# eldenpark/halo2-pse

Hardware: AMD Instinct MI355X
Metric: bn254_msm_g1_adds_per_sec (higher is better)
Workload: dtype u32x8 (256-bit Montgomery integers)

## Files before the change

### halo2-pse_amd/csrc/api.hip

```cpp
#include <dlfcn.h>
#include <rccl/rccl.h>
#include <stdarg.h>
#include <stdlib.h>
#include <string.h>

#include <atomic>
#include <condition_variable>
#include <deque>
#include <functional>
#include <shared_mutex>
#include <thread>

#include "../../include/halo2hip.h"
#include "../../include/halo2hip_debug.h"
#include "engine.h"

extern "C" {
static void lazy_forget(const void* key);
static void lazy_reset();
static void lazy_pin_consider(const uint64_t* bases_xy, size_t n);
}

namespace h2 {

static thread_local char g_err[512] = "";

void set_error(const char* fmt, ...) {
    va_list ap;
    va_start(ap, fmt);
    vsnprintf(g_err, sizeof(g_err), fmt, ap);
    va_end(ap);
}

int DevBuf::ensure(size_t bytes) {
    if (bytes <= cap) return 0;
    if (p) {
        H2_CHECK(hipDeviceSynchronize());
        H2_CHECK(hipFree(p));
// ... 169 lines not shown
            for (auto& w : mask_ac) w = 0xffffffffu;
            for (auto& w : mask_b) w = 0xffffffffu;
        }
        H2_CHECK(hipExtStreamCreateWithCUMask(&aux1, words, mask_ac.data()));
        H2_CHECK(hipExtStreamCreateWithCUMask(&aux2, words, mask_ac.data()));
        H2_CHECK(hipExtStreamCreateWithCUMask(&aux_b, words, mask_b.data()));
        aux_reserved = K;
    }
    while (aux_events.size() < n_events) {
        hipEvent_t e;
        H2_CHECK(hipEventCreateWithFlags(&e, hipEventDisableTiming));
        aux_events.push_back(e);
    }
    return 0;
}

struct Config {
    size_t multi_gpu_min_n = (size_t)1 << 18;
    size_t msm_min_n = (size_t)1 << 10;
    uint32_t ntt_min_log_n = 10;
    bool gather_rccl = false;
    bool fixed_base = true;
    size_t table_max_bytes = (size_t)160 << 30;
    bool allow_dup = false;
    bool roctx = false;
    uint32_t lazy_pin_after = 0;
    size_t column_cache_bytes = (size_t)64 << 30;
};
static Config g_cfg;

static bool env_u64(const char* name, uint64_t* out) {
    const char* v = getenv(name);
    if (!v || !*v) return false;
    char* end = nullptr;
    unsigned long long x = strtoull(v, &end, 0);
    if (end == v) return false;
    *out = x;
    return true;
}

static void read_config() {
    Config c;
    uint64_t v;
    if (env_u64("HALO2_HIP_MULTI_GPU_MIN_N", &v)) c.multi_gpu_min_n = (size_t)v;
    if (env_u64("HALO2_HIP_MSM_MIN_N", &v)) c.msm_min_n = (size_t)v;
    if (env_u64("HALO2_HIP_NTT_MIN_LOGN", &v)) c.ntt_min_log_n = (uint32_t)v;
    if (env_u64("HALO2_HIP_FIXED_BASE", &v)) c.fixed_base = v != 0;
    if (env_u64("HALO2_HIP_TABLE_MAX_GB", &v)) c.table_max_bytes = (size_t)v << 30;
    if (env_u64("HALO2_HIP_ALLOW_DUPLICATE_DEVICES", &v)) c.allow_dup = v != 0;
    if (env_u64("HALO2_HIP_ROCTX", &v)) c.roctx = v != 0;
    if (env_u64("HALO2_HIP_LAZY_PIN", &v)) c.lazy_pin_after = (uint32_t)v;
    if (env_u64("HALO2_HIP_COLUMN_CACHE_GB", &v)) c.column_cache_bytes = (size_t)v << 30;
    if (env_u64("HALO2_HIP_NTT_TWIDDLE_MB", &v)) ntt_set_full_twiddle_budget(v << 20);
    if (env_u64("HALO2_HIP_EVALH_CODEGEN", &v)) evalh_debug_set_codegen((int)v, 0);
    if (env_u64("HALO2_HIP_MSM_WINDOW", &v) && v >= 2 && v <= 24) msm_set_window((uint32_t)v);
    {
        uint64_t on = 1, min_n = 0;
        const bool has_on = env_u64("HALO2_HIP_STREAM", &on), has_min = env_u64("HALO2_HIP_STREAM_MIN_N", &min_n);
        if (has_on || has_min) msm_set_stream(has_on && on == 0 ? 1 : 0, 0.0, has_min ? (size_t)min_n : 0);
    }
    const char* g = getenv("HALO2_HIP_GATHER");
    if (g && !strcmp(g, "rccl")) c.gather_rccl = true;
    g_cfg = c;
}

static int (*g_roctx_push)(const char*) = nullptr;
static int (*g_roctx_pop)() = nullptr;
static void roctx_load() {
    if (g_roctx_push) return;
    void* h = dlopen("libroctx64.so.4", RTLD_NOW | RTLD_GLOBAL);
    if (!h) h = dlopen("libroctx64.so", RTLD_NOW | RTLD_GLOBAL);
    if (!h) return;
    g_roctx_push = (int (*)(const char*))dlsym(h, "roctxRangePushA");
    g_roctx_pop = (int (*)())dlsym(h, "roctxRangePop");
    if (!g_roctx_push || !g_roctx_pop) g_roctx_push = nullptr, g_roctx_pop = nullptr;
}

struct Rccl {
// ... 631 lines not shown
            const size_t i = pin_sample_index(total, k);
            if (i < n) ok = memcmp(it->second.sample + 64 * k, bases_xy + 8 * i, 64) == 0;
        }
    }
    if (!ok) {
        ::lazy_forget((const void*)bases_xy);
        (void)unpin_everywhere((const void*)bases_xy);
        return true;
    }
    return n == total || n > pin_sample_index(total, 3);
}

__global__ void pin_sample_kernel(const Affine* __restrict__ src, size_t total, Affine* __restrict__ out) {
    if (threadIdx.x < H2_PIN_SAMPLES) out[threadIdx.x] = src[pin_sample_index(total, threadIdx.x)];
}

static const MsmTable* pinned_table(Ctx* c, const void* key, size_t n, MsmTable* out, const PinnedBases** entry) {
    auto it = c->pinned.find(key);
    if (it == c->pinned.end() || !it->second.device_key || n > it->second.n || !it->second.c) return nullptr;
    out->table = (const Affine*)it->second.d;
    out->stride = it->second.n;
    out->c = it->second.c;
    out->W = it->second.W;
    *entry = &it->second;
    return out;
}

static int msm_device_keyed(Ctx* c, const Fe* const* d_scalars, const Affine* d_bases, size_t n, size_t count, XYZZ* out, hipStream_t s) {
    MsmTable tab;
    const PinnedBases* pb = nullptr;
    const MsmTable* t = (n && count) ? pinned_table(c, d_bases, n, &tab, &pb) : nullptr;
    if (t && n != pb->n && n <= pin_sample_index(pb->n, 3)) t = nullptr;
    volatile uint32_t* flag = nullptr;
    if (t && pb->d_sample) {
        int rc = c->pin_flag.ensure(64);
        if (rc) return rc;
        flag = (volatile uint32_t*)c->pin_flag.p;
        *flag = 0;
        c->pin_chk.bases = d_bases;
        c->pin_chk.samples = (const Affine*)pb->d_sample;
        c->pin_chk.flag = (uint32_t*)c->pin_flag.p;
        c->pin_chk.n = n;
        c->pin_chk.total = pb->n;
    }
    int rc = msm_batch_device(c, d_scalars, false, d_bases, n, count, out, s, t);
    c->pin_chk = Ctx::PinCheck();
// ... 103 lines not shown
    const Fe* sc = (const Fe*)d_scalars;
    int rc = msm_device_keyed(en.c, &sc, (const Affine*)d_bases_xy, n, 1, &r, s);
    if (rc) return rc;
    xyzz_to_out(r, out_xyz);
    return 0;
}

static int msm_shard_host(Ctx* c, const uint64_t* const* scalars, const uint64_t* bases_xy, size_t lo, size_t n, size_t count, XYZZ* out,
                          bool use_cache = true) {
    std::vector<const Fe*> sc(count);
    for (size_t j = 0; j < count; j++) sc[j] = (const Fe*)scalars[j] + lo;
    MsmTable tab;
    const Affine *d_bases = nullptr, *h_bases = nullptr;
    const MsmTable* t = nullptr;
    auto it = c->pinned.find((const void*)bases_xy);
    if (use_cache && it != c->pinned.end() && it->second.lo <= lo && lo + n <= it->second.hi) {
        const PinnedBases& pb = it->second;
        d_bases = (const Affine*)pb.d + (lo - pb.lo);
        if (pb.c) {
            tab.table = d_bases;
            tab.stride = pb.n;
            tab.c = pb.c;
            tab.W = pb.W;
            t = &tab;
        }
    } else {
        h_bases = (const Affine*)bases_xy + lo;
    }
    return msm_batch_device(c, sc.data(), true, d_bases, n, count, out, c->stream, t, h_bases);
}

static void fold_host(int n_use, size_t count, const std::vector<std::vector<XYZZ>>& parts, uint64_t* out_xyz) {
    for (size_t j = 0; j < count; j++) {
        XYZZ acc = xyzz_identity();
        for (int d = 0; d < n_use; d++) xyzz_add(acc, parts[(size_t)d][j]);
        xyzz_to_out(acc, out_xyz + 12 * j);
    }
}

static int gather_rccl(size_t count, std::vector<XYZZ>* all) {
    const int nd = (int)g_devs.size();
    const size_t bytes = count * sizeof(XYZZ);
    if (g_rccl.comms.size() != (size_t)nd || bytes > H2_GATHER_OWN) return H2HIP_EINVAL;
    ncclResult_t nr = g_rccl.GroupStart();
    for (int d = 0; nr == ncclSuccess && d < nd; d++) {
        Ctx* x = g_devs[(size_t)d];
// ... 129 lines not shown
    if (rc) return rc;
    for (size_t j = 0; j < count; j++) xyzz_to_out(r[j], out_xyz + 12 * j);
    return 0;
}

static int pin_on_device(Ctx* c, const void* key, const uint64_t* h_points, const void* d_src, size_t lo, size_t hi, size_t n_total,
                         const uint8_t* sample, bool device_key) {
    (void)n_total;
    auto it = c->pinned.find(key);
    if (it != c->pinned.end()) {
        H2_CHECK(hipDeviceSynchronize());
        (void)hipFree(it->second.d);
        if (it->second.d_sample) (void)hipFree(it->second.d_sample);
        c->pinned.erase(it);
    }
    if (hi <= lo) return 0;
    const size_t n = hi - lo;
    PinnedBases pb;
    pb.n = n;
    pb.lo = lo;
    pb.hi = hi;
    pb.device_key = device_key;
    if (sample) memcpy(pb.sample, sample, sizeof(pb.sample));
    uint32_t cw = 0, W = 1;
    if (g_cfg.fixed_base && n <= ((size_t)1 << 26)) {
        cw = msm_table_window(n);
        W = (255 + cw - 1) / cw;
        if ((size_t)W * n * sizeof(Affine) > g_cfg.table_max_bytes) cw = 0, W = 1;
    }
    hipError_t e = hipMalloc(&pb.d, (size_t)W * n * sizeof(Affine));
    if (e != hipSuccess && cw) {
        (void)hipGetLastError();
        cw = 0;
        W = 1;
        e = hipMalloc(&pb.d, n * sizeof(Affine));
    }
    if (e != hipSuccess) {
        set_error("bases_pin: hipMalloc(%zu) failed: %s", (size_t)W * n * sizeof(Affine), hipGetErrorString(e));
        return H2HIP_ENOMEM;
    }
    int rc = 0;
    if (d_src) {
        if (!cw) H2_CHECK(hipMemcpyAsync(pb.d, (const Affine*)d_src + lo, n * sizeof(Affine), hipMemcpyDeviceToDevice, c->stream));
    } else {
        H2_CHECK(hipMemcpyAsync(pb.d, (const Affine*)h_points + lo, n * sizeof(Affine), hipMemcpyHostToDevice, c->stream));
    }
    if (cw) rc = msm_table_build(c, d_src ? (const Affine*)d_src + lo : (const Affine*)pb.d, n, cw, (Affine*)pb.d, c->stream);
    if (!rc && device_key) {
        if (hipMalloc(&pb.d_sample, H2_PIN_SAMPLES * sizeof(Affine)) != hipSuccess) {
            (void)hipGetLastError();
            pb.d_sample = nullptr;
            set_error("bases_pin: hipMalloc of the fingerprint failed");
            rc = H2HIP_ENOMEM;
        } else {
            hipLaunchKernelGGL(pin_sample_kernel, dim3(1), dim3(64), 0, c->stream, (const Affine*)d_src + lo, n, (Affine*)pb.d_sample);
        }
    }
    if (!rc && hipStreamSynchronize(c->stream) != hipSuccess) {
        set_error("bases_pin: table build failed");
        rc = H2HIP_EDEVICE;
    }
    if (rc) {
        (void)hipFree(pb.d);
        if (pb.d_sample) (void)hipFree(pb.d_sample);
        return rc;
    }
    pb.c = cw;
    pb.W = cw ? W : 0;
    c->pinned[key] = pb;
    return 0;
}

static void pin_sample(const uint64_t* bases_xy, size_t n, uint8_t* out) {
    for (uint32_t k = 0; k < H2_PIN_SAMPLES; k++) memcpy(out + 64 * k, bases_xy + 8 * pin_sample_index(n, k), 64);
}

static int pin_host_everywhere(const uint64_t* bases_xy, size_t n) {
    uint8_t sample[H2_PIN_SAMPLES * 64];
    pin_sample(bases_xy, n, sample);
    const int nd = (int)g_devs.size();
    const int use = n >= g_cfg.multi_gpu_min_n ? nd : 1;
    const size_t per = n / (size_t)use;
    int rc = on_devices(nd, [&](int d) -> int {
        size_t lo = d < use ? (size_t)d * per : n, hi = d < use ? (d == use - 1 ? n : (size_t)(d + 1) * per) : n;
        return pin_on_device(g_devs[(size_t)d], (const void*)bases_xy, bases_xy, nullptr, lo, hi, n, sample, false);
    });
    if (rc) (void)unpin_everywhere((const void*)bases_xy);
    return rc;
}

int h2hip_bases_pin(const uint64_t* bases_xy, size_t n) {
// ... 147 lines not shown
        return 0;
    });
    if (rc) return rc;
    std::vector<XYZZ> all;
    if ((rc = gather_rccl(count, &all))) return rc;
    std::vector<std::vector<XYZZ>> parts((size_t)nd, std::vector<XYZZ>(count));
    for (int d = 0; d < nd; d++)
        for (size_t j = 0; j < count; j++) parts[(size_t)d][j] = all[(size_t)d * count + j];
    fold_host(nd, count, parts, out_xyz);
    return 0;
}

int h2hip_bases_pinned_info(const void* bases_xy, size_t* n_points, uint32_t* window_bits, uint32_t* windows, size_t* device_bytes) {
    Entry en(nullptr, nullptr, true);
    if (en.rc) return en.rc;
    size_t n = 0, bytes = 0;
    uint32_t c = 0, W = 0;
    bool found = false;
    for (Ctx* x : g_devs) {
        auto it = x->pinned.find(bases_xy);
        if (it == x->pinned.end()) continue;
        found = true;
        n += it->second.n;
        bytes += (size_t)(it->second.c ? it->second.W : 1) * it->second.n * sizeof(Affine);
        if (it->second.c) c = it->second.c, W = it->second.W;
    }
    if (!found) {
        set_error("bases_pinned_info: pointer is not pinned");
        return H2HIP_EINVAL;
    }
    if (n_points) *n_points = n;
    if (window_bits) *window_bits = c;
    if (windows) *windows = W;
    if (device_bytes) *device_bytes = bytes;
    return 0;
}

int h2hip_g1_fold(const uint64_t* partials_xyz, size_t k, uint64_t out_xyz[12]) {
    if (!out_xyz || (k && !partials_xyz)) {
        set_error("g1_fold: null argument");
        return H2HIP_EINVAL;
    }
    XYZZ acc = xyzz_identity();
    for (size_t i = 0; i < k; i++) {
        Jac j;
        memcpy(&j, partials_xyz + 12 * i, 96);
        xyzz_add(acc, jac_to_xyzz(j));
    }
// ... 590 lines not shown
        return H2HIP_EINVAL;
    }
    Entry en("h2hip_gen_scalars_device", d_out);
    if (en.rc) return en.rc;
    return gen_scalars_device(seed, start, n, (Fe*)d_out, (hipStream_t)stream);
}

int h2hip_gen_points_device(uint64_t seed, uint64_t start, size_t n, void* d_out, void* stream) {
    if (n && !d_out) {
        set_error("gen_points: null output");
        return H2HIP_EINVAL;
    }
    Entry en("h2hip_gen_points_device", d_out);
    if (en.rc) return en.rc;
    return gen_points_device(seed, start, n, (Affine*)d_out, (hipStream_t)stream);
}

int h2hip_set_msm_window(uint32_t c) {
    if (c != 0 && (c < 2 || c > 24)) {
        set_error("msm window must be 0 (auto) or 2..24");
        return H2HIP_EINVAL;
    }
    msm_set_window(c);
    return 0;
}

uint32_t h2hip_get_msm_window(size_t n) { return msm_get_window(n); }
uint32_t h2hip_get_msm_window_fixed_base(size_t n) { return msm_table_window(n); }

int h2hip_debug_set_msm_max_chunk(size_t m) {
    msm_set_max_chunk(m);
    return 0;
}

int h2hip_debug_set_msm_stream(uint32_t chunks, uint32_t ratio_permille, size_t min_n) {
    msm_set_stream(chunks, ratio_permille / 1000.0, min_n);
    return 0;
}

size_t h2hip_debug_msm_stream_ladder(size_t n, uint32_t chunks, uint32_t ratio_permille, int with_bases, size_t* sizes, size_t cap) {
    if (!sizes && cap) return 0;
    return msm_debug_ladder(n, chunks, ratio_permille / 1000.0, with_bases != 0, sizes, cap);
}

int h2hip_debug_set_msm_heavy_div(size_t d) {
    msm_set_heavy_div(d);
    return 0;
}

int h2hip_debug_set_g2l_quad(int on) {
    ecfft_set_quad(on != 0);
// ... 167 lines not shown
```

### halo2-pse_amd/csrc/engine.h

```cpp
#pragma once
#include <hip/hip_runtime.h>
#include <stdint.h>
#include <stdio.h>
#include <string.h>

#include <map>
#include <mutex>
#include <shared_mutex>
#include <string>
#include <vector>

#include "../../include/halo2hip.h"
#include "ecu.h"

namespace h2 {

void set_error(const char* fmt, ...);

#define H2_CHECK(expr)                                                                             \
    do {                                                                                           \
        hipError_t _e = (expr);                                                                    \
        if (_e != hipSuccess) {                                                                    \
            h2::set_error("%s:%d: %s -> %s", __FILE__, __LINE__, #expr, hipGetErrorString(_e));    \
            return 2;                                                                              \
// ... 21 lines not shown
        for (int i = 0; i < 8; i++)
            if (omega[i] != o.omega[i]) return omega[i] < o.omega[i];
        return log_n < o.log_n;
    }
};

struct TwiddleTable {
    Fu* lo = nullptr;
    Fu* hi = nullptr;
    uint32_t lo_bits = 0;
    Fu* stage_of[13] = {};
#define H2_TW_FULL 12
    Fu* full[H2_TW_FULL] = {};
    uint32_t full_tag[H2_TW_FULL] = {};
    Fe full_scale[H2_TW_FULL] = {};
    Fu* lo_scaled = nullptr;
    Fe lo_scale;
};

struct MsmTable {
    const Affine* table = nullptr;
    size_t stride = 0;
    uint32_t c = 0, W = 0;
};

#define H2_GATHER_OWN ((size_t)64 << 10)
#define H2_PIN_SAMPLES 16
static inline __host__ __device__ size_t pin_sample_index(size_t total, uint32_t k) { return k == 0 ? 0 : (total - 1) >> (H2_PIN_SAMPLES - 1 - k); }
struct PinnedBases {
    void* d = nullptr;
    size_t n = 0;
    uint32_t c = 0, W = 0;
    bool device_key = false;
    uint8_t sample[H2_PIN_SAMPLES * 64];
    void* d_sample = nullptr;
    size_t lo = 0, hi = 0;
};

struct Ctx;

#define H2_COL_SAMPLES 16
struct PinnedColumn {
    void* d = nullptr;
    size_t elems = 0;
    uint64_t last_use = 0;
    uint8_t sample[H2_COL_SAMPLES * 32];
};

struct StageTimer {
    std::string name;
    hipEvent_t e0 = nullptr, e1 = nullptr;
    double total_ms = 0.0;
    uint64_t count = 0;
    bool pending = false;
};
// ... 287 lines not shown
```

### halo2-pse_amd/csrc/msm.hip

```cpp
#include <hip/hip_ext.h>
#include <string.h>

#include <atomic>
#include <condition_variable>
#include <thread>
#include <vector>

#include "ecq.h"
#include "engine.h"
#include "host64.h"

namespace h2 {

#define MSM_MAX_C1 1024u
#define MSM_MAX_L 12u
#define MSM_STAGE 16384u
#define MSM_COUNT_TILE 4096u

struct MsmPlan {
    uint32_t c;
    uint32_t W;
    uint32_t q;
    uint32_t cb;
    uint32_t NB;
    uint32_t shared;
    uint32_t heavy_t;
    uint32_t chunk;
};

template <class F>
__device__ __forceinline__ void for_each_digit(const Fe& s, uint32_t c, uint32_t q, uint32_t W, F&& f) {
    uint64_t buf = 0;
    uint32_t nb = 0, w = 0, carry = 0;
    uint32_t width = q ? c : c - 1;
    auto emit = [&]() {
        uint32_t d = ((uint32_t)buf & ((1u << width) - 1)) + carry;
        uint32_t neg = 0;
        carry = 0;
        if (d > (1u << (width - 1))) {
            d = (1u << width) - d;
            neg = 1;
            carry = 1;
        }
        if (d) f(w, d - 1, neg);
        w++;
        buf >>= width;
        nb = nb > width ? nb - width : 0;
        width = w < q ? c : c - 1;
    };
#pragma unroll
    for (int limb = 0; limb < 8; limb++) {
        buf |= (uint64_t)s.l[limb] << nb;
        nb += 32;
        while (nb >= width && w < W) emit();
    }
    while (w < W) emit();
}

struct L1Args {
    const Fe* scalars_one;
    const Fe* const* list;
    uint32_t n, c, q, W, cb, L, C1;
    uint32_t shared, stride;
    uint32_t tile;
    uint16_t* tile_hist;
    const uint32_t* tile_off;
    uint2* tmp;
    uint32_t* tmp_e;
    uint16_t* tmp_k;
    const Affine* chk_bases;
    const Affine* chk_samples;
    uint32_t* chk_flag;
    size_t chk_n, chk_total;
};

__device__ __forceinline__ Fe fr_to_canonical(const Fe& x) {
    Fu c32 = fu_zero();
    c32.l[0] = 32;
    return fu_mul_canon<FrU>(fu_slice(x), c32);
}

#define MSM_TCHUNK 64u
#ifndef MSM_SCATTER_XG
#define MSM_SCATTER_XG 4u
#endif

__global__ void __launch_bounds__(256) msm_l1_count_kernel(L1Args a) {
    __shared__ uint32_t lh[MSM_MAX_C1];
    if (a.chk_flag && blockIdx.x == 0 && blockIdx.y == 0 && threadIdx.x < 4 * H2_PIN_SAMPLES) {
        const uint32_t k = threadIdx.x >> 2, part = threadIdx.x & 3;
        const size_t idx = pin_sample_index(a.chk_total, k);
        if (idx < a.chk_n) {
            const uint4 u = reinterpret_cast<const uint4*>(&a.chk_bases[idx])[part], v = reinterpret_cast<const uint4*>(&a.chk_samples[k])[part];
            if (u.x != v.x || u.y != v.y || u.z != v.z || u.w != v.w) atomicOr(a.chk_flag, 1u);
        }
    }
    for (uint32_t b = threadIdx.x; b < a.C1; b += 256) lh[b] = 0;
    __syncthreads();
    const Fe* __restrict__ scalars = a.list ? a.list[blockIdx.y] : a.scalars_one;
    const uint32_t set0 = a.shared ? blockIdx.y : blockIdx.y * a.W;
    for (uint32_t t = threadIdx.x; t < a.tile; t += 256) {
        const uint32_t i = blockIdx.x * a.tile + t;
        if (i < a.n) {
            const Fe sc = fr_to_canonical(scalars[i]);
            for_each_digit(sc, a.c, a.q, a.W, [&](uint32_t w, uint32_t slot, uint32_t) {
                const uint32_t gb = ((set0 + (a.shared ? 0u : w)) << a.cb) | slot;
                atomicAdd(&lh[gb >> a.L], 1u);
            });
        }
    }
    __syncthreads();
    uint16_t* row = a.tile_hist + (size_t)(blockIdx.y * gridDim.x + blockIdx.x) * a.C1;
    for (uint32_t b = threadIdx.x; b < a.C1; b += 256) row[b] = (uint16_t)lh[b];
}

__global__ void __launch_bounds__(256) msm_l1_chunk_kernel(const uint16_t* __restrict__ tile_hist, uint32_t n_tiles, uint32_t C1,
                                                           uint32_t* __restrict__ chunk_sum) {
    const uint32_t b = blockIdx.y * 256 + threadIdx.x;
    if (b >= C1) return;
    const uint32_t t0 = blockIdx.x * MSM_TCHUNK, t1 = t0 + MSM_TCHUNK < n_tiles ? t0 + MSM_TCHUNK : n_tiles;
    uint32_t sum = 0;
#pragma unroll 8
    for (uint32_t t = t0; t < t1; t++) sum += tile_hist[(size_t)t * C1 + b];
    chunk_sum[(size_t)blockIdx.x * C1 + b] = sum;
}

template <int BS>
__device__ __forceinline__ uint32_t block_scan_base(const uint32_t* cnt, uint32_t n, uint32_t per, uint32_t* ps, uint32_t* total) {
// ... 33 lines not shown
    uint32_t tx = blockIdx.x;
    if (XG && tx < (gridDim.x & ~((8u << XG) - 1))) {
        const uint32_t q = tx >> (3 + XG), r = tx & ((8u << XG) - 1);
        tx = ((q * 8 + (r & 7)) << XG) | (r >> 3);
    }
    const size_t row = (size_t)(blockIdx.y * gridDim.x + tx) * a.C1;
    for (uint32_t b = threadIdx.x; b < a.C1; b += 1024) cur[b] = a.tile_hist[row + b];
    const Fe* __restrict__ scalars = a.list ? a.list[blockIdx.y] : a.scalars_one;
    const uint32_t set0 = a.shared ? blockIdx.y : blockIdx.y * a.W;
    const uint32_t i = tx * a.tile + threadIdx.x;
    const bool live = threadIdx.x < a.tile && i < a.n;
    Fe sc;
    if (live) sc = fr_to_canonical(scalars[i]);
    __syncthreads();
    uint32_t total;
    uint32_t run = block_scan_base<1024>(cur, a.C1, 1, ps, &total);
    if (threadIdx.x < a.C1) {
        const uint32_t b = threadIdx.x;
        delta[b] = a.tile_off[row + b] - run;
        cur[b] = run;
    }
    __syncthreads();
    if (live) {
        for_each_digit(sc, a.c, a.q, a.W, [&](uint32_t w, uint32_t slot, uint32_t neg) {
            const uint32_t gb = ((set0 + (a.shared ? 0u : w)) << a.cb) | slot;
            const uint32_t pos = atomicAdd(&cur[gb >> a.L], 1u);
            stage[pos] = make_uint2((a.shared ? w * a.stride + i : i) | (neg << 31), gb);
        });
    }
    __syncthreads();
    for (uint32_t pos = threadIdx.x; pos < total; pos += 1024) {
        const uint2 e = stage[pos];
        const uint32_t at = pos + delta[e.y >> a.L];
        if (SPLIT) {
            a.tmp_e[at] = e.x;
            a.tmp_k[at] = (uint16_t)(e.y & ((1u << a.L) - 1));
        } else {
            a.tmp[at] = e;
        }
    }
}

__global__ void __launch_bounds__(1024) msm_l1_scan_kernel(uint32_t* __restrict__ chunk_sum, uint32_t n_chunks, uint32_t C1,
                                                           uint32_t* __restrict__ bin_total, uint32_t* __restrict__ zero, uint32_t zero_words) {
    __shared__ uint32_t part_sum[16][64];
    if (blockIdx.x == 0)
        for (uint32_t i = threadIdx.x; i < zero_words; i += 1024) zero[i] = 0;
    const uint32_t lb = threadIdx.x & 63, p = threadIdx.x >> 6, b = blockIdx.x * 64 + lb;
    const uint32_t per = (n_chunks + 15) / 16, c0 = p * per, c1 = c0 + per < n_chunks ? c0 + per : n_chunks;
    uint32_t sum = 0;
// ... 517 lines not shown
    }
    if (live && g == 0) J.out[task] = sh[threadIdx.x];
}

struct FinalArr {
    const XYZZu* base;
    uint32_t stride;
    uint32_t len;
    uint32_t o, k;
    uint32_t nbits;
};
struct FinalArgs {
    FinalArr arr[4];
    uint32_t n_arr;
};

__global__ void __launch_bounds__(256) msm_final_kernel(FinalArgs args, XYZZ* __restrict__ set_sums) {
    __shared__ XYZZu sh[256];
    const uint32_t set = blockIdx.x, ai = threadIdx.x >> 6, v = threadIdx.x & 63;
    XYZZu x = xyzzu_identity();
    if (ai < args.n_arr) {
        const FinalArr& A = args.arr[ai];
        if (v < A.len) {
            const uint32_t wgt = (v + A.o) << A.k;
            if (wgt) x = xyzzu_mul_small(A.base[(size_t)set * A.stride + v], wgt, A.nbits);
        }
    }
    XYZZu r = block_tree_sum(x, sh);
    if (threadIdx.x == 0) set_sums[set] = xyzzu_to_ext(r);
}


__global__ void __launch_bounds__(64) msm_rowcol_quad_kernel(RowColArgs args) {
    __shared__ XYZZu sh[16];
    uint32_t ji = 0;
    for (uint32_t q = 1; q < args.n_jobs; q++)
        if (blockIdx.x >= args.job[q].first_block) ji = q;
    const RowColJob& J = args.job[ji];
    const uint32_t quad = threadIdx.x >> 2, role = threadIdx.x & 3;
    const uint32_t G = 1u << J.g_log, g = quad & (G - 1);
    const uint32_t rows = 1u << J.log_rows, cols = 1u << J.log_cols;
    const uint32_t per_arr = J.cols_kind ? cols : rows;
    const uint32_t task = (blockIdx.x - J.first_block) * (16u >> J.g_log) + (quad >> J.g_log);
    const bool live = task < J.n_arr * per_arr;
    XYZZu acc = xyzzu_identity();
    if (live) {
        const uint32_t a = task / per_arr, idx = task - a * per_arr;
// ... 26 lines not shown
    const uint32_t set = blockIdx.x / n_groups, group = blockIdx.x - set * n_groups;
    const uint32_t quad = threadIdx.x >> 2, role = threadIdx.x & 3;
    uint32_t e = group * 16 + quad;
    const XYZZu* base = nullptr;
    uint32_t stride = 0, o = 0, k = 0, nbits = 0;
    bool found = false;
#pragma unroll
    for (uint32_t i = 0; i < 4; i++) {
        if (i < args.n_arr && !found) {
            if (e < args.arr[i].len) {
                found = true;
                base = args.arr[i].base;
                stride = args.arr[i].stride;
                o = args.arr[i].o;
                k = args.arr[i].k;
                nbits = args.arr[i].nbits;
            } else {
                e -= args.arr[i].len;
            }
        }
    }
    XYZZu x = xyzzu_identity();
    if (found) {
        const uint32_t wgt = (e + o) << k;
        if (wgt) x = xyzzu_mul_small_q(base[(size_t)set * stride + e], wgt, nbits, role);
    }
    if (role == 0) sh[quad] = x;
    __syncthreads();
    for (uint32_t st = 8; st >= 1; st >>= 1) {
        if (quad < st) {
            XYZZu a = sh[quad];
            xyzzu_add_q(a, sh[quad + st], role);
            if (role == 0) sh[quad] = a;
        }
        __syncthreads();
    }
    if (n_groups == 1) {
        if (threadIdx.x == 0) set_sums[set] = xyzzu_to_ext(sh[0]);
        return;
    }
    if (threadIdx.x == 0) {
        partials[blockIdx.x] = sh[0];
        __threadfence();
        is_last = atomicAdd(&done[set], 1u) == n_groups - 1;
    }
    __syncthreads();
    if (!is_last) return;
// ... 18 lines not shown
struct PlaneJob {
    const XYZZu* base;
    uint32_t log_len;
    uint32_t o;
    uint32_t n_planes;
    uint32_t wgs;
    uint32_t first_plane;
    uint32_t first_block;
};
struct PlaneArgs {
    PlaneJob job[2];
    uint32_t blocks_per_set, planes_per_set;
};

__global__ void __launch_bounds__(256) msm_planes_kernel(PlaneArgs args, XYZZu* __restrict__ partials, uint32_t* __restrict__ done,
                                                         XYZZ* __restrict__ plane_sums) {
    __shared__ XYZZu sh[64];
    __shared__ uint32_t is_last;
    const uint32_t set = blockIdx.x / args.blocks_per_set, b = blockIdx.x - set * args.blocks_per_set;
    const PlaneJob& J = args.job[b >= args.job[1].first_block ? 1 : 0];
    const uint32_t pb = b - J.first_block, plane = pb / J.wgs, part = pb - plane * J.wgs;
    const XYZZu* X = J.base + ((size_t)set << J.log_len);
    const uint32_t quad = threadIdx.x >> 2, role = threadIdx.x & 3;
    const bool top = plane == J.log_len;
    const uint32_t count = top ? 1u : 1u << (J.log_len - 1);
    auto elem = [&](uint32_t t) -> XYZZu {
        if (t >= count) return xyzzu_identity();
        const uint32_t v = top ? (1u << J.log_len) : ((t >> plane) << (plane + 1)) | (1u << plane) | (t & ((1u << plane) - 1));
        return X[v - J.o];
    };
    const uint32_t t0 = part * 128 + 2 * quad;
    const XYZZu x = xyzzu_sum_q(elem(t0), elem(t0 + 1), role);
    if (role == 0) sh[quad] = x;
    __syncthreads();
    for (uint32_t st = 32; st >= 1; st >>= 1) {
        if (quad < st) {
            const XYZZu a = xyzzu_sum_q(sh[quad], sh[quad + st], role);
            if (role == 0) sh[quad] = a;
        }
        __syncthreads();
    }
    const uint32_t out = set * args.planes_per_set + J.first_plane + plane;
    if (J.wgs == 1) {
        if (threadIdx.x == 0) plane_sums[out] = xyzzu_to_ext(sh[0]);
        return;
    }
    if (threadIdx.x == 0) {
        partials[(size_t)out * 16 + part] = sh[0];
        __threadfence();
        is_last = atomicAdd(&done[out], 1u) == J.wgs - 1;
    }
    __syncthreads();
    if (!is_last) return;
    __builtin_amdgcn_fence(__ATOMIC_ACQUIRE, "agent");
    XYZZu y = xyzzu_identity();
// ... 63 lines not shown
    if (lg <= 8) return 7;
    if (lg <= 12) return 10;
    if (lg <= 14) return 13;
    if (lg <= 17) return 15;
    return 17;
}

static uint32_t normalise_window(uint32_t c) {
    if (c < 2) c = 2;
    if (c > 22) c = 22;
    const uint32_t W = (255 + c - 1) / c;
    return (255 + W - 1) / W;
}

uint32_t msm_table_window(size_t n) {
    if (g_window_override) return normalise_window(g_window_override);
    const uint32_t lg = floor_log2(n);
    uint32_t c = lg <= 12 ? 13 : lg <= 17 ? 17 : lg <= 21 ? 20 : 22;
    return normalise_window(c);
}

static MsmPlan make_plan(size_t n, bool fused, const MsmTable* tab, uint32_t force_c = 0) {
    MsmPlan p;
    uint32_t c = tab ? tab->c : force_c ? force_c : plain_window(n, fused);
    if (c < 2) c = 2;
    if (c > 24) c = 24;
    p.W = (255 + c - 1) / c;
    c = (255 + p.W - 1) / p.W;
    p.c = c;
    p.q = 255 - p.W * (c - 1);
    p.cb = c - 1;
    p.NB = 1u << (c - 1);
    p.shared = tab ? 1 : 0;
    size_t t = (n * p.W) / g_heavy_div;
    if (t < 32) t = 32;
    const size_t mean = (p.shared ? n * p.W : n) >> p.cb;
    if (t < 8 * mean) t = 8 * mean;
    p.heavy_t = (uint32_t)t;
    p.chunk = 1024;
    return p;
}

uint32_t msm_get_window(size_t n) { return make_plan(n, false, nullptr).c; }

static XYZZ combine_windows(const XYZZ* ws, const MsmPlan& p) {
    h64::P acc = h64::identity();
// ... 22 lines not shown
    MsmPlan p;
    size_t n, E;
    uint32_t K;
    uint32_t L, C1, bin_shift;
    uint32_t tile, tiles_x, n_tiles, n_tchunks;
    uint32_t split_log;
    uint32_t levels, s, rb, s2, s3;
    size_t max_chunks, max_heavy;
    size_t o_zero, o_zero_end, o_bintot, o_hist, o_hcnt, o_fdone, o_cstart, o_tmp, o_vals, o_start, o_counts, o_perm, o_buckets, o_parts, o_RA, o_CA, o_RR,
        o_RC, o_CR, o_CC, o_sums, o_partials, o_ppart, o_hb, o_hc, o_hs, o_ptrs, o_thist, o_toff, o_chsum, total;
};

static int msm_layout(size_t n, MsmLayout* L, uint32_t fuse, const MsmTable* tab, uint32_t force_c = 0, int force_split = -1) {
    MsmPlan p = make_plan(n, fuse > 1, tab, force_c);
    L->p = p;
    L->n = n;
    L->fuse = fuse;
    L->n_sets = p.shared ? fuse : fuse * p.W;
    L->E = n * p.W * fuse;
    if (L->E >= ((size_t)1 << 31)) {
        set_error("msm: %zu entries exceed the 2^31 limit of one run (window override too small?)", L->E);
        return 1;
    }
    if (p.shared && (uint64_t)p.W * tab->stride >= (1ull << 31)) {
        set_error("msm: fixed-base table index exceeds 31 bits");
        return 1;
    }
    const uint64_t K64 = (uint64_t)L->n_sets << p.cb;
    if (K64 > ((uint64_t)MSM_MAX_C1 << MSM_MAX_L)) {
        set_error("msm: too many buckets (%llu) for one run", (unsigned long long)K64);
        return 1;
    }
    L->K = (uint32_t)K64;
    uint32_t want = 1;
    while (want < MSM_MAX_C1 && (size_t)want * g_bin_entries < L->E) want <<= 1;
    uint32_t Lb = 0;
    while (Lb < p.cb && Lb < MSM_MAX_L && (K64 >> Lb) > want) Lb++;
    while ((K64 >> Lb) > MSM_MAX_C1) {
        if (Lb >= p.cb || Lb >= MSM_MAX_L) {
            set_error("msm: too many bucket sets (%u) for one run", L->n_sets);
            return 1;
        }
        Lb++;
    }
    L->L = Lb;
    L->C1 = (uint32_t)(K64 >> Lb);
    L->tile = (MSM_STAGE / p.W) & ~63u;
// ... 58 lines not shown
    const MsmPlan& p = L.p;
    const size_t n = L.n;
    uint32_t* cstart = (uint32_t*)(base + L.o_cstart);
    uint32_t *vals = (uint32_t*)(base + L.o_vals), *start = (uint32_t*)(base + L.o_start);
    uint32_t *counts = (uint32_t*)(base + L.o_counts), *perm = (uint32_t*)(base + L.o_perm);
    int t0 = c->timer_begin("msm_digits", s);
    L1Args a;
    a.scalars_one = d_scalars_list[0];
    a.list = nullptr;
    if (L.fuse > 1) {
        int rc = c->stage_h2d(base + L.o_ptrs, d_scalars_list, L.fuse * sizeof(void*), s);
        if (rc) return rc;
        a.list = (const Fe* const*)(base + L.o_ptrs);
    }
    a.n = (uint32_t)n;
    a.c = p.c;
    a.q = p.q;
    a.W = p.W;
    a.cb = p.cb;
    a.L = L.L;
    a.C1 = L.C1;
    a.shared = p.shared;
    a.stride = tab ? (uint32_t)tab->stride : 0;
    a.tile = L.tile;
    a.tile_hist = (uint16_t*)(base + L.o_thist);
    a.tile_off = (const uint32_t*)(base + L.o_toff);
    a.tmp = (uint2*)(base + L.o_tmp);
    a.chk_bases = c->pin_chk.bases;
    a.chk_samples = c->pin_chk.samples;
    a.chk_flag = c->pin_chk.flag;
    a.chk_n = c->pin_chk.n;
    a.chk_total = c->pin_chk.total;
    c->pin_chk = Ctx::PinCheck();
    uint32_t* chsum = (uint32_t*)(base + L.o_chsum);
    const dim3 tiles(L.tiles_x, L.fuse), chunks(L.n_tchunks, (L.C1 + 255) / 256);
    hipLaunchKernelGGL(msm_l1_count_kernel, tiles, dim3(256), 0, s, a);
    H2_CHECK(hipGetLastError());
    c->timer_end(t0, s);
    int t1 = c->timer_begin("msm_sort", s);
    hipLaunchKernelGGL(msm_l1_chunk_kernel, chunks, dim3(256), 0, s, (const uint16_t*)a.tile_hist, L.n_tiles, L.C1, chsum);
    H2_CHECK(hipGetLastError());
    uint32_t* bin_total = (uint32_t*)(base + L.o_bintot);
    hipLaunchKernelGGL(msm_l1_scan_kernel, dim3((L.C1 + 63) / 64), dim3(1024), 0, s, chsum, L.n_tchunks, L.C1, bin_total,
                       (uint32_t*)(base + L.o_zero), (uint32_t)((L.o_zero_end - L.o_zero) / 4));
    H2_CHECK(hipGetLastError());
    hipLaunchKernelGGL(msm_l1_offsets_kernel, chunks, dim3(256), 0, s, (const uint16_t*)a.tile_hist, L.n_tiles, L.C1, (const uint32_t*)chsum,
// ... 77 lines not shown
        j->log_cols = log_cols;
        j->cols_kind = kind;
        j->g_log = g_log;
        j->first_block = *n_blocks;
        const uint64_t tasks = (uint64_t)n_arr << log_sums;
        const uint32_t per_block = (quad ? 16u : 256u) >> g_log;
        *n_blocks += (uint32_t)((tasks + per_block - 1) / per_block);
    }
}

static bool g_plane_tail = true;
void msm_set_plane_tail(bool on) { g_plane_tail = on; }
static bool msm_plane_tail(const Ctx* c, const MsmLayout& L) {
    return g_plane_tail && g_quad_tail && L.levels >= 1 && L.n_sets <= MSM_PLANE_SETS_MAX && L.rb <= 11 && L.s <= 11 && L.rb >= 1 && L.s >= 1 &&
           L.s + 1 + L.rb <= MSM_PLANES_MAX && !c->gather_want;
}
static inline uint32_t msm_planes_per_set(const MsmLayout& L) { return L.rb + L.s + 1; }

static void msm_planes_finish(const MsmLayout& L, const XYZZ* planes, XYZZ* sums) {
    const uint32_t pps = msm_planes_per_set(L);
    for (uint32_t set = 0; set < L.n_sets; set++) {
        const XYZZ* P = planes + (size_t)set * pps;
        h64::P acc = h64::identity();
        for (uint32_t m = L.s + L.rb; m-- > 0;) {
            acc = h64::pdouble(acc);
            if (m >= L.s) h64::padd(acc, h64::from_xyzz(P[L.s + 1 + (m - L.s)]));
            if (m <= L.s) h64::padd(acc, h64::from_xyzz(P[m]));
        }
        sums[set] = h64::to_xyzz(acc);
    }
}

static int msm_stage_c(Ctx* c, const MsmLayout& L, char* base, XYZZ* h_sums, hipStream_t s, XYZZ* h_planes = nullptr) {
    XYZZu* buckets = (XYZZu*)(base + L.o_buckets);
    XYZZu *RA = (XYZZu*)(base + L.o_RA), *CA = (XYZZu*)(base + L.o_CA), *RR = (XYZZu*)(base + L.o_RR), *RC = (XYZZu*)(base + L.o_RC);
    XYZZu *CR = (XYZZu*)(base + L.o_CR), *CC = (XYZZu*)(base + L.o_CC);
    const bool direct = !c->gather_want;
    XYZZ* sums = direct ? h_sums : (XYZZ*)(base + L.o_sums);
    const uint32_t ns = L.n_sets, cb = L.p.cb;
    const bool quad = g_quad_tail && ns <= 64;
    int t4 = c->timer_begin("msm_reduce", s);
    FinalArgs fa;
    memset(&fa, 0, sizeof(fa));
    auto set_arr = [&](uint32_t i, const XYZZu* b, uint32_t log_len, uint32_t o, uint32_t k) {
        fa.arr[i].base = b;
        fa.arr[i].stride = 1u << log_len;
        fa.arr[i].len = 1u << log_len;
        fa.arr[i].o = o;
        fa.arr[i].k = k;
        fa.arr[i].nbits = bits_of(((1u << log_len) - 1 + o) << k);
    };
    if (L.levels == 0) {
        set_arr(0, buckets, cb, 1, 0);
        fa.n_arr = 1;
    } else {
        RowColArgs ra;
        memset(&ra, 0, sizeof(ra));
        uint32_t nblk = 0;
        rowcol_jobs(&ra, buckets, RA, CA, ns, L.rb, L.s, &nblk);
        if (g_rowcol_qtree)
            hipLaunchKernelGGL(msm_rowcol_qtree_kernel<FqUA>, dim3(nblk), dim3(256), 0, s, ra);
        else if (g_rowcol_asm)
            hipLaunchKernelGGL(msm_rowcol_kernel<FqUA>, dim3(nblk), dim3(256), 0, s, ra);
        else
            hipLaunchKernelGGL(msm_rowcol_kernel<FqU>, dim3(nblk), dim3(256), 0, s, ra);
        H2_CHECK(hipGetLastError());
        if (h_planes && msm_plane_tail(c, L)) {
            PlaneArgs pa;
            memset(&pa, 0, sizeof(pa));
            uint32_t blk = 0, pl = 0;
            for (uint32_t k = 0; k < 2; k++) {
                PlaneJob& J = pa.job[k];
                J.base = k ? RA : CA;
                J.log_len = k ? L.rb : L.s;
                J.o = k ? 0 : 1;
                J.n_planes = J.log_len + J.o;
                J.wgs = J.log_len > 7 ? 1u << (J.log_len - 8) : 1;
                J.first_plane = pl;
                J.first_block = blk;
                pl += J.n_planes;
                blk += J.n_planes * J.wgs;
            }
            pa.blocks_per_set = blk;
            pa.planes_per_set = pl;
            hipLaunchKernelGGL(msm_planes_kernel, dim3(ns * blk), dim3(256), 0, s, pa, (XYZZu*)(base + L.o_ppart), (uint32_t*)(base + L.o_fdone), h_planes);
            H2_CHECK(hipGetLastError());
            c->timer_end(t4, s);
            return 0;
        }
        if (L.levels == 1) {
            set_arr(0, RA, L.rb, 0, L.s);
            set_arr(1, CA, L.s, 1, 0);
            fa.n_arr = 2;
        } else {
            memset(&ra, 0, sizeof(ra));
            nblk = 0;
            rowcol_jobs(&ra, RA, RR, RC, ns, L.rb - L.s2, L.s2, &nblk, quad);
            rowcol_jobs(&ra, CA, CR, CC, ns, L.s - L.s3, L.s3, &nblk, quad);
            if (quad)
// ... 443 lines not shown
```

### include/halo2hip_debug.h

```cpp
#ifndef HALO2HIP_DEBUG_H
#define HALO2HIP_DEBUG_H
#include "halo2hip.h"

#ifdef __cplusplus
extern "C" {
#endif

int h2hip_debug_set_msm_stream(uint32_t chunks, uint32_t ratio_permille, size_t min_n);
size_t h2hip_debug_msm_stream_ladder(size_t n, uint32_t chunks, uint32_t ratio_permille, int with_bases, size_t* sizes, size_t cap);
int h2hip_debug_set_msm_max_chunk(size_t m);
int h2hip_debug_rccl_gather_selftest(const uint64_t* partials_xyz, size_t count, uint64_t* out_xyz);
int h2hip_debug_set_msm_heavy_div(size_t d);
int h2hip_debug_set_g2l_quad(int on);
int h2hip_debug_set_msm_fuse_limits(size_t entries, size_t max_n);
int h2hip_debug_set_msm_rowcol(uint64_t lanes, int use_asm);
int h2hip_debug_set_msm_split_buckets(int on);
int h2hip_debug_set_msm_plane_tail(int on);
int h2hip_debug_set_msm_quad_tail(int on);
int h2hip_debug_set_msm_bucket_order(int local);
int h2hip_debug_set_msm_split_records(int on);
int h2hip_debug_set_msm_bin_entries(size_t d);
int h2hip_debug_set_reserved_cus(uint32_t k);
int h2hip_debug_set_msm_fuse_small(int on);
int h2hip_debug_set_ntt_smax(uint32_t v);
int h2hip_debug_ntt_plan(uint32_t log_n, size_t count, uint32_t radices[4]);
int h2hip_debug_set_lazy_pin(uint32_t after);
int h2hip_debug_set_ntt_two_pass(uint32_t lo, uint32_t hi);
int h2hip_debug_set_ntt_twiddle_budget(uint64_t bytes);
int h2hip_debug_set_ntt_batch_bytes(uint64_t bytes);
int h2hip_debug_set_ntt_two_pass_batch_wgs(uint64_t v);
int h2hip_debug_set_ntt_full_max_log_m(uint32_t v);
int h2hip_debug_set_ntt_fold_tables(int on);
int h2hip_debug_set_ntt_host_batch(uint64_t run_bytes, uint64_t group_bytes);
int h2hip_debug_set_ntt_two_pass_log_j(int v);
int h2hip_debug_set_evalh_max_local_slots(uint32_t v);
int h2hip_debug_set_evalh_lookup_group_bytes(uint64_t v);
int h2hip_debug_evalh_program_muls(const h2hip_graph* g, uint32_t* n_mul);
int h2hip_debug_set_evalh_codegen(int mode, uint32_t max_ops);
int h2hip_debug_evalh_codegen_source(const h2hip_graph* g, char* buf, size_t cap, size_t* len, int compile, double* seconds, size_t* code_bytes);
int h2hip_debug_evalh_codegen_stats(uint64_t out[5]);
int h2hip_debug_evalh_compile_stats(const h2hip_graph* g, uint32_t* n_ops, uint32_t* n_slots);
int h2hip_debug_set_opening_tile(uint32_t rows_per_thread, uint32_t threads_per_tile);
int h2hip_debug_set_lookup_sort(uint32_t lds_keys);
int h2hip_debug_lookup_sort_stats(uint32_t out[2]);
// ... 7 lines not shown
```

Before: 11.59 billion.

## Add per-bit fixed-base table with sliding-window NAF digit decomposition for MSM

For pinned bases with n between 2^19 and 2^23, a 255-row table of 2^k·P is built and scalars are recoded as signed odd-digit sliding-window NAF. Each nonzero digit maps to a bucket by its odd magnitude and to a table row by its bit position. All digits share one bucket set of 2^(w-2) odd buckets with width 20 by default, and the final bucket reduction and plane kernels are adjusted for odd weights. This aims to cut the number of bucket adds per scalar by skipping zero runs and to shrink the reduction, but it costs a much larger table in memory and allocation, with more gather traffic.

```diff
diff --git a/halo2-pse_amd/csrc/api.hip b/halo2-pse_amd/csrc/api.hip
--- a/halo2-pse_amd/csrc/api.hip
+++ b/halo2-pse_amd/csrc/api.hip
@@ -14,6 +14,7 @@
 #include "../../include/halo2hip.h"
 #include "../../include/halo2hip_debug.h"
 #include "engine.h"
+#include "msm_naf.h"
 
 extern "C" {
 static void lazy_forget(const void* key);
@@ -229,12 +230,23 @@
     bool gather_rccl = false;
     bool fixed_base = true;
     size_t table_max_bytes = (size_t)160 << 30;
+    size_t bit_table_max_bytes = (size_t)40 << 30;
     bool allow_dup = false;
     bool roctx = false;
     uint32_t lazy_pin_after = 0;
     size_t column_cache_bytes = (size_t)64 << 30;
 };
 static Config g_cfg;
+
+static uint32_t g_window_req = 0;
+static int g_bit_min_log = 19;
+static uint32_t g_bit_w = 0;
+static uint32_t bit_table_naf(size_t n) {
+    if (g_bit_min_log < 0 || g_bit_min_log > 23 || n < ((size_t)1 << g_bit_min_log) || n > ((size_t)1 << 23)) return 0;
+    if ((size_t)H2_BIT_TABLE_ROWS * n * sizeof(Affine) > g_cfg.bit_table_max_bytes) return 0;
+    const uint32_t w = g_bit_w ? g_bit_w : g_window_req ? g_window_req : msm_naf_default_width(n);
+    return w < 3 ? 3 : w > 22 ? 22 : w;
+}
 
 static bool env_u64(const char* name, uint64_t* out) {
     const char* v = getenv(name);
@@ -254,13 +266,14 @@
     if (env_u64("HALO2_HIP_NTT_MIN_LOGN", &v)) c.ntt_min_log_n = (uint32_t)v;
     if (env_u64("HALO2_HIP_FIXED_BASE", &v)) c.fixed_base = v != 0;
     if (env_u64("HALO2_HIP_TABLE_MAX_GB", &v)) c.table_max_bytes = (size_t)v << 30;
+    if (env_u64("HALO2_HIP_BIT_TABLE_MAX_GB", &v)) c.bit_table_max_bytes = (size_t)v << 30;
     if (env_u64("HALO2_HIP_ALLOW_DUPLICATE_DEVICES", &v)) c.allow_dup = v != 0;
     if (env_u64("HALO2_HIP_ROCTX", &v)) c.roctx = v != 0;
     if (env_u64("HALO2_HIP_LAZY_PIN", &v)) c.lazy_pin_after = (uint32_t)v;
     if (env_u64("HALO2_HIP_COLUMN_CACHE_GB", &v)) c.column_cache_bytes = (size_t)v << 30;
     if (env_u64("HALO2_HIP_NTT_TWIDDLE_MB", &v)) ntt_set_full_twiddle_budget(v << 20);
     if (env_u64("HALO2_HIP_EVALH_CODEGEN", &v)) evalh_debug_set_codegen((int)v, 0);
-    if (env_u64("HALO2_HIP_MSM_WINDOW", &v) && v >= 2 && v <= 24) msm_set_window((uint32_t)v);
+    if (env_u64("HALO2_HIP_MSM_WINDOW", &v) && v >= 2 && v <= 24) msm_set_window((uint32_t)v), g_window_req = (uint32_t)v;
     {
         uint64_t on = 1, min_n = 0;
         const bool has_on = env_u64("HALO2_HIP_STREAM", &on), has_min = env_u64("HALO2_HIP_STREAM_MIN_N", &min_n);
@@ -938,6 +951,7 @@
     out->stride = it->second.n;
     out->c = it->second.c;
     out->W = it->second.W;
+    out->naf = it->second.naf;
     *entry = &it->second;
     return out;
 }
@@ -1087,6 +1101,7 @@
             tab.stride = pb.n;
             tab.c = pb.c;
             tab.W = pb.W;
+            tab.naf = pb.naf;
             t = &tab;
         }
     } else {
@@ -1262,21 +1277,35 @@
     pb.hi = hi;
     pb.device_key = device_key;
     if (sample) memcpy(pb.sample, sample, sizeof(pb.sample));
-    uint32_t cw = 0, W = 1;
+    uint32_t cw = 0, W = 1, naf = 0, rows = 1;
     if (g_cfg.fixed_base && n <= ((size_t)1 << 26)) {
         cw = msm_table_window(n);
-        W = (255 + cw - 1) / cw;
-        if ((size_t)W * n * sizeof(Affine) > g_cfg.table_max_bytes) cw = 0, W = 1;
-    }
-    hipError_t e = hipMalloc(&pb.d, (size_t)W * n * sizeof(Affine));
+        rows = W = (255 + cw - 1) / cw;
+        if ((size_t)W * n * sizeof(Affine) > g_cfg.table_max_bytes) cw = 0, rows = W = 1;
+        if (cw && (naf = bit_table_naf(n))) {
+            size_t held = 0;
+            for (const auto& kv : c->pinned) held += (size_t)(kv.second.naf ? H2_BIT_TABLE_ROWS : kv.second.c ? kv.second.W : 1) * kv.second.n * sizeof(Affine);
+            if (held + (size_t)H2_BIT_TABLE_ROWS * n * sizeof(Affine) > g_cfg.table_max_bytes)
+                naf = 0;
+            else
+                rows = H2_BIT_TABLE_ROWS;
+        }
+    }
+    hipError_t e = hipMalloc(&pb.d, (size_t)rows * n * sizeof(Affine));
+    if (e != hipSuccess && naf) {
+        (void)hipGetLastError();
+        naf = 0;
+        rows = W;
+        e = hipMalloc(&pb.d, (size_t)rows * n * sizeof(Affine));
+    }
     if (e != hipSuccess && cw) {
         (void)hipGetLastError();
         cw = 0;
-        W = 1;
+        rows = W = 1;
         e = hipMalloc(&pb.d, n * sizeof(Affine));
     }
     if (e != hipSuccess) {
-        set_error("bases_pin: hipMalloc(%zu) failed: %s", (size_t)W * n * sizeof(Affine), hipGetErrorString(e));
+        set_error("bases_pin: hipMalloc(%zu) failed: %s", (size_t)rows * n * sizeof(Affine), hipGetErrorString(e));
         return H2HIP_ENOMEM;
     }
     int rc = 0;
@@ -1285,7 +1314,7 @@
     } else {
         H2_CHECK(hipMemcpyAsync(pb.d, (const Affine*)h_points + lo, n * sizeof(Affine), hipMemcpyHostToDevice, c->stream));
     }
-    if (cw) rc = msm_table_build(c, d_src ? (const Affine*)d_src + lo : (const Affine*)pb.d, n, cw, (Affine*)pb.d, c->stream);
+    if (cw) rc = msm_table_build(c, d_src ? (const Affine*)d_src + lo : (const Affine*)pb.d, n, naf ? 1 : cw, (Affine*)pb.d, c->stream);
     if (!rc && device_key) {
         if (hipMalloc(&pb.d_sample, H2_PIN_SAMPLES * sizeof(Affine)) != hipSuccess) {
             (void)hipGetLastError();
@@ -1307,6 +1336,7 @@
     }
     pb.c = cw;
     pb.W = cw ? W : 0;
+    pb.naf = naf;
     c->pinned[key] = pb;
     return 0;
 }
@@ -1500,8 +1530,12 @@
         if (it == x->pinned.end()) continue;
         found = true;
         n += it->second.n;
-        bytes += (size_t)(it->second.c ? it->second.W : 1) * it->second.n * sizeof(Affine);
-        if (it->second.c) c = it->second.c, W = it->second.W;
+        const PinnedBases& pb = it->second;
+        bytes += (size_t)(pb.naf ? H2_BIT_TABLE_ROWS : pb.c ? pb.W : 1) * pb.n * sizeof(Affine);
+        if (pb.naf)
+            c = pb.naf, W = (255 + pb.naf - 1) / pb.naf;
+        else if (pb.c)
+            c = pb.c, W = pb.W;
     }
     if (!found) {
         set_error("bases_pinned_info: pointer is not pinned");
@@ -2138,11 +2172,25 @@
         return H2HIP_EINVAL;
     }
     msm_set_window(c);
+    g_window_req = c;
     return 0;
 }
 
 uint32_t h2hip_get_msm_window(size_t n) { return msm_get_window(n); }
-uint32_t h2hip_get_msm_window_fixed_base(size_t n) { return msm_table_window(n); }
+uint32_t h2hip_get_msm_window_fixed_base(size_t n) {
+    const uint32_t naf = g_cfg.fixed_base ? bit_table_naf(n) : 0;
+    return naf ? naf : msm_table_window(n);
+}
+
+int h2hip_debug_set_msm_bit_table(int min_log_n, uint32_t w) {
+    if (w != 0 && (w < 3 || w > 22)) {
+        set_error("msm bit table: width must be 0 (auto) or 3..22");
+        return H2HIP_EINVAL;
+    }
+    g_bit_min_log = min_log_n == 0 ? 19 : min_log_n;
+    g_bit_w = w;
+    return 0;
+}
 
 int h2hip_debug_set_msm_max_chunk(size_t m) {
     msm_set_max_chunk(m);
diff --git a/halo2-pse_amd/csrc/engine.h b/halo2-pse_amd/csrc/engine.h
--- a/halo2-pse_amd/csrc/engine.h
+++ b/halo2-pse_amd/csrc/engine.h
@@ -67,7 +67,9 @@
     const Affine* table = nullptr;
     size_t stride = 0;
     uint32_t c = 0, W = 0;
-};
+    uint32_t naf = 0;
+};
+#define H2_BIT_TABLE_ROWS 255u
 
 #define H2_GATHER_OWN ((size_t)64 << 10)
 #define H2_PIN_SAMPLES 16
@@ -76,6 +78,7 @@
     void* d = nullptr;
     size_t n = 0;
     uint32_t c = 0, W = 0;
+    uint32_t naf = 0;
     bool device_key = false;
     uint8_t sample[H2_PIN_SAMPLES * 64];
     void* d_sample = nullptr;
diff --git a/halo2-pse_amd/csrc/msm.hip b/halo2-pse_amd/csrc/msm.hip
--- a/halo2-pse_amd/csrc/msm.hip
+++ b/halo2-pse_amd/csrc/msm.hip
@@ -9,6 +9,7 @@
 #include "ecq.h"
 #include "engine.h"
 #include "host64.h"
+#include "msm_naf.h"
 
 namespace h2 {
 
@@ -24,6 +25,7 @@
     uint32_t cb;
     uint32_t NB;
     uint32_t shared;
+    uint32_t naf;
     uint32_t heavy_t;
     uint32_t chunk;
 };
@@ -62,6 +64,7 @@
     const Fe* const* list;
     uint32_t n, c, q, W, cb, L, C1;
     uint32_t shared, stride;
+    uint32_t naf, bit_rows;
     uint32_t tile;
     uint16_t* tile_hist;
     const uint32_t* tile_off;
@@ -74,6 +77,17 @@
     size_t chk_n, chk_total;
 };
 
+template <class F>
+__device__ __forceinline__ void for_each_entry(const Fe& s, const L1Args& a, F&& f) {
+    if (a.naf) {
+        for_each_naf_digit(s, a.naf, [&](uint32_t pos, uint32_t slot, uint32_t neg) { f(0u, pos, slot, neg); });
+    } else {
+        for_each_digit(s, a.c, a.q, a.W, [&](uint32_t w, uint32_t slot, uint32_t neg) {
+            f(w, a.bit_rows ? w * (a.c - 1) + (w < a.q ? w : a.q) : w, slot, neg);
+        });
+    }
+}
+
 __device__ __forceinline__ Fe fr_to_canonical(const Fe& x) {
     Fu c32 = fu_zero();
     c32.l[0] = 32;
@@ -103,7 +117,7 @@
         const uint32_t i = blockIdx.x * a.tile + t;
         if (i < a.n) {
             const Fe sc = fr_to_canonical(scalars[i]);
-            for_each_digit(sc, a.c, a.q, a.W, [&](uint32_t w, uint32_t slot, uint32_t) {
+            for_each_entry(sc, a, [&](uint32_t w, uint32_t, uint32_t slot, uint32_t) {
                 const uint32_t gb = ((set0 + (a.shared ? 0u : w)) << a.cb) | slot;
                 atomicAdd(&lh[gb >> a.L], 1u);
             });
@@ -183,10 +197,10 @@
     }
     __syncthreads();
     if (live) {
-        for_each_digit(sc, a.c, a.q, a.W, [&](uint32_t w, uint32_t slot, uint32_t neg) {
+        for_each_entry(sc, a, [&](uint32_t w, uint32_t row, uint32_t slot, uint32_t neg) {
             const uint32_t gb = ((set0 + (a.shared ? 0u : w)) << a.cb) | slot;
             const uint32_t pos = atomicAdd(&cur[gb >> a.L], 1u);
-            stage[pos] = make_uint2((a.shared ? w * a.stride + i : i) | (neg << 31), gb);
+            stage[pos] = make_uint2((a.shared ? row * a.stride + i : i) | (neg << 31), gb);
         });
     }
     __syncthreads();
@@ -750,7 +764,7 @@
     if (ai < args.n_arr) {
         const FinalArr& A = args.arr[ai];
         if (v < A.len) {
-            const uint32_t wgt = (v + A.o) << A.k;
+            const uint32_t wgt = (v << A.k) + A.o;
             if (wgt) x = xyzzu_mul_small(A.base[(size_t)set * A.stride + v], wgt, A.nbits);
         }
     }
@@ -823,7 +837,7 @@
     }
     XYZZu x = xyzzu_identity();
     if (found) {
-        const uint32_t wgt = (e + o) << k;
+        const uint32_t wgt = (e << k) + o;
         if (wgt) x = xyzzu_mul_small_q(base[(size_t)set * stride + e], wgt, nbits, role);
     }
     if (role == 0) sh[quad] = x;
@@ -888,15 +902,17 @@
     const uint32_t pb = b - J.first_block, plane = pb / J.wgs, part = pb - plane * J.wgs;
     const XYZZu* X = J.base + ((size_t)set << J.log_len);
     const uint32_t quad = threadIdx.x >> 2, role = threadIdx.x & 3;
-    const bool top = plane == J.log_len;
-    const uint32_t count = top ? 1u : 1u << (J.log_len - 1);
+    const bool top = J.o == 1 && plane == J.log_len, all = J.o == 2 && plane == 0;
+    const uint32_t bit = J.o == 2 ? plane - 1 : plane;
+    const uint32_t count = top ? 1u : all ? 1u << J.log_len : 1u << (J.log_len - 1);
     auto elem = [&](uint32_t t) -> XYZZu {
         if (t >= count) return xyzzu_identity();
-        const uint32_t v = top ? (1u << J.log_len) : ((t >> plane) << (plane + 1)) | (1u << plane) | (t & ((1u << plane) - 1));
-        return X[v - J.o];
+        const uint32_t v = top ? (1u << J.log_len) : all ? t : ((t >> bit) << (bit + 1)) | (1u << bit) | (t & ((1u << bit) - 1));
+        return X[v - (J.o & 1)];
     };
-    const uint32_t t0 = part * 128 + 2 * quad;
-    const XYZZu x = xyzzu_sum_q(elem(t0), elem(t0 + 1), role);
+    const uint32_t t0 = all ? part * 256 + 4 * quad : part * 128 + 2 * quad;
+    XYZZu x = xyzzu_sum_q(elem(t0), elem(t0 + 1), role);
+    if (all) x = xyzzu_sum_q(x, xyzzu_sum_q(elem(t0 + 2), elem(t0 + 3), role), role);
     if (role == 0) sh[quad] = x;
     __syncthreads();
     for (uint32_t st = 32; st >= 1; st >>= 1) {
@@ -1006,6 +1022,23 @@
 
 static MsmPlan make_plan(size_t n, bool fused, const MsmTable* tab, uint32_t force_c = 0) {
     MsmPlan p;
+    p.naf = 0;
+    if (tab && tab->naf && !fused) {
+        const uint32_t w = tab->naf;
+        p.naf = p.c = w;
+        p.W = (255 + w - 1) / w;
+        p.q = 0;
+        p.cb = w - 2;
+        p.NB = 1u << p.cb;
+        p.shared = 1;
+        size_t t = (n * p.W) / g_heavy_div;
+        if (t < 32) t = 32;
+        const size_t mean = (n * p.W) >> p.cb;
+        if (t < 8 * mean) t = 8 * mean;
+        p.heavy_t = (uint32_t)t;
+        p.chunk = 1024;
+        return p;
+    }
     uint32_t c = tab ? tab->c : force_c ? force_c : plain_window(n, fused);
     if (c < 2) c = 2;
     if (c > 24) c = 24;
@@ -1074,7 +1107,7 @@
         set_error("msm: %zu entries exceed the 2^31 limit of one run (window override too small?)", L->E);
         return 1;
     }
-    if (p.shared && (uint64_t)p.W * tab->stride >= (1ull << 31)) {
+    if (p.shared && (uint64_t)(tab->naf ? H2_BIT_TABLE_ROWS : p.W) * tab->stride >= (1ull << 31)) {
         set_error("msm: fixed-base table index exceeds 31 bits");
         return 1;
     }
@@ -1179,6 +1212,8 @@
     a.C1 = L.C1;
     a.shared = p.shared;
     a.stride = tab ? (uint32_t)tab->stride : 0;
+    a.naf = p.naf;
+    a.bit_rows = tab && tab->naf ? 1 : 0;
     a.tile = L.tile;
     a.tile_hist = (uint16_t*)(base + L.o_thist);
     a.tile_off = (const uint32_t*)(base + L.o_toff);
@@ -1302,6 +1337,14 @@
     for (uint32_t set = 0; set < L.n_sets; set++) {
         const XYZZ* P = planes + (size_t)set * pps;
         h64::P acc = h64::identity();
+        if (L.p.naf) {
+            for (uint32_t m = L.s + L.rb + 1; m-- > 0;) {
+                acc = h64::pdouble(acc);
+                h64::padd(acc, h64::from_xyzz(P[m]));
+            }
+            sums[set] = h64::to_xyzz(acc);
+            continue;
+        }
         for (uint32_t m = L.s + L.rb; m-- > 0;) {
             acc = h64::pdouble(acc);
             if (m >= L.s) h64::padd(acc, h64::from_xyzz(P[L.s + 1 + (m - L.s)]));
@@ -1322,13 +1365,15 @@
     int t4 = c->timer_begin("msm_reduce", s);
     FinalArgs fa;
     memset(&fa, 0, sizeof(fa));
+    const uint32_t odd = L.p.naf ? 1 : 0;
     auto set_arr = [&](uint32_t i, const XYZZu* b, uint32_t log_len, uint32_t o, uint32_t k) {
+        k += odd;
         fa.arr[i].base = b;
         fa.arr[i].stride = 1u << log_len;
         fa.arr[i].len = 1u << log_len;
         fa.arr[i].o = o;
         fa.arr[i].k = k;
-        fa.arr[i].nbits = bits_of(((1u << log_len) - 1 + o) << k);
+        fa.arr[i].nbits = bits_of((((1u << log_len) - 1) << k) + o);
     };
     if (L.levels == 0) {
         set_arr(0, buckets, cb, 1, 0);
@@ -1353,8 +1398,8 @@
                 PlaneJob& J = pa.job[k];
                 J.base = k ? RA : CA;
                 J.log_len = k ? L.rb : L.s;
-                J.o = k ? 0 : 1;
-                J.n_planes = J.log_len + J.o;
+                J.o = k ? 0 : 1 + odd;
+                J.n_planes = J.log_len + (k ? 0 : 1);
                 J.wgs = J.log_len > 7 ? 1u << (J.log_len - 8) : 1;
                 J.first_plane = pl;
                 J.first_block = blk;
diff --git a/halo2-pse_amd/csrc/msm_naf.h b/halo2-pse_amd/csrc/msm_naf.h
--- /dev/null
+++ b/halo2-pse_amd/csrc/msm_naf.h
@@ -0,0 +1,46 @@
+#pragma once
+#include "field.h"
+
+namespace h2 {
+
+template <class F>
+H2_HD void for_each_naf_digit(const Fe& s, uint32_t w, F&& f) {
+    uint64_t buf = 0;
+    uint32_t nb = 0, pos = 0, carry = 0;
+    const uint32_t mask = (1u << w) - 1, half = 1u << (w - 1);
+    auto drain = [&]() {
+        for (;;) {
+            const uint64_t t = carry ? ~buf : buf;
+            uint32_t skip = t ? (uint32_t)__builtin_ctzll(t) : 64u;
+            if (skip > nb) skip = nb;
+            buf >>= skip;
+            nb -= skip;
+            pos += skip;
+            if (nb < w) return;
+            const uint32_t x = ((uint32_t)buf & mask) + carry;
+            carry = x > half ? 1u : 0u;
+            const uint32_t mag = carry ? (1u << w) - x : x;
+            f(pos, (mag - 1) >> 1, carry);
+            buf >>= w;
+            nb -= w;
+            pos += w;
+        }
+    };
+#pragma unroll
+    for (int limb = 0; limb < 8; limb++) {
+        buf |= (uint64_t)s.l[limb] << nb;
+        nb += 32;
+        drain();
+    }
+    do {
+        nb += 32;
+        drain();
+    } while (buf || carry);
+}
+
+static inline uint32_t msm_naf_default_width(size_t n) {
+    (void)n;
+    return 20;
+}
+
+}
diff --git a/include/halo2hip_debug.h b/include/halo2hip_debug.h
--- a/include/halo2hip_debug.h
+++ b/include/halo2hip_debug.h
@@ -20,6 +20,7 @@
 int h2hip_debug_set_msm_bucket_order(int local);
 int h2hip_debug_set_msm_split_records(int on);
 int h2hip_debug_set_msm_bin_entries(size_t d);
+int h2hip_debug_set_msm_bit_table(int min_log_n, uint32_t w);
 int h2hip_debug_set_reserved_cus(uint32_t k);
 int h2hip_debug_set_msm_fuse_small(int on);
 int h2hip_debug_set_ntt_smax(uint32_t v);
```

Result: slower. 4.544 billion (-60.8%).
